# ViliamVadocz/takzero

Hardware: AMD Instinct MI355X
Metric: mcts_simulations_per_s (higher is better)
Workload: dtype f16

## Files before the change

takzero_amd/csrc/tz_capi.hip:

```cpp
#include <algorithm>
#include <array>
#include <cmath>
#include <cstdlib>
#include <cstring>
#include <vector>

#include "tz_math.h"
#include "tz_nn.h"

struct tz_search {
    SearchDev d;
    tz_net* net = nullptr;
    int device = 0;
    hipStream_t stream = nullptr;
    bool own_stream = false;
    float* noise_dev = nullptr;
    int noise_cap = 0;
    uint16_t* act_dev = nullptr;
    int32_t* i32_dev = nullptr;
    int8_t* i8_dev = nullptr;
    tz_root_info* info_dev = nullptr;
    void* child_dev = nullptr;
    size_t child_cap = 0;
    hipGraphExec_t graph[2] = {nullptr, nullptr};
// ... 106 lines not shown
            if (s->net) s->net->profile = v;
        }
    } restore{s, saved_net_profile};
    if (profile) {
        TZ_HIP(hipEventCreate(&e0));
        TZ_HIP(hipEventCreate(&e1));
        TZ_HIP(hipEventCreate(&e2));
        TZ_HIP(hipEventCreate(&e3));
        TZ_HIP(hipEventRecord(e0, s->stream));
    }
    if ((rc = tz_tree_descend(s->d, from_start, s->stream))) return rc;
    if ((rc = tz_tree_compact_leaves(s->d, s->stream))) return rc;
    if (profile) TZ_HIP(hipEventRecord(e1, s->stream));
    NetOut out{nullptr, 0, nullptr, nullptr};
    if (s->d.agent_kind == TZ_AGENT_NET) {
        if ((rc = tz_net_forward_device(s->net, s->d.leaf_env, s->d.nn_game, s->d.nn_count, 0, s->d.batch, s->stream, &out)))
            return rc;
    }
    if (profile) TZ_HIP(hipEventRecord(e2, s->stream));
    if ((rc = tz_tree_expand(s->d, out, s->stream))) return rc;
    if (profile) {
        TZ_HIP(hipEventRecord(e3, s->stream));
        s->tree_events.push_back({e0, e1});
        s->tree_events.push_back({e2, e3});
        s->steps++;
    }
    return TZ_OK;
}

int ensure_noise(tz_search* s, int amax) {
    if ((size_t)amax * s->d.batch <= (size_t)s->noise_cap) return TZ_OK;
// ... 742 lines not shown
```

takzero_amd/csrc/tz_engine.h:

```cpp
#pragma once
#include <hip/hip_runtime.h>
#include <stdint.h>

#include <string>
#include <vector>

#include "../../include/takzero_hip.h"

#define TZ_MAX_DEPTH 512

void tz_set_error(const std::string& msg);
int tz_fail(int code, const std::string& msg);
#define TZ_HIP(call)                                                                              \
    do {                                                                                          \
        hipError_t _e = (call);                                                                   \
        if (_e != hipSuccess)                                                                     \
            return tz_fail(TZ_EDEVICE, std::string(#call) + ": " + hipGetErrorString(_e));       \
    } while (0)

struct TreeArrays {
    uint8_t* eval_tag;
    uint32_t* eval_bits;
    uint32_t* visits;
    float* prob;
// ... 40 lines not shown
    float* prob;
    float* value;
    float* variance;
    uint8_t* bad;
    int32_t* count;
    int32_t* forwards;
    int32_t* offset;
    int32_t* index;
};

struct NetOut {
    const float* policy;
    int policy_stride;
    const float* value;
    const float* variance;
};

int tz_tree_descend(const SearchDev& s, bool from_start_nodes, hipStream_t st);
int tz_tree_compact_leaves(const SearchDev& s, hipStream_t st);
int tz_tree_expand(const SearchDev& s, const NetOut& out, hipStream_t st);
int tz_tree_apply_noise(const SearchDev& s, const float* noise_dev, int amax, float ratio, hipStream_t st);
int tz_tree_root_info(const SearchDev& s, tz_root_info* out_dev, hipStream_t st);
int tz_tree_root_children(const SearchDev& s, int amax, uint16_t* move_idx, uint32_t* visits, uint8_t* eval_tag,
                          uint32_t* eval_bits, float* logit, float* prob, float* std_dev, hipStream_t st);
int tz_tree_node(const SearchDev& s, int game, const uint16_t* path_dev, int len, uint32_t* out_words, int* status, int amax,
                 uint16_t* move_idx, uint32_t* visits, uint8_t* eval_tag, uint32_t* eval_bits, float* logit, float* prob, float* std_dev,
                 hipStream_t st);
int tz_tree_select_best(const SearchDev& s, uint16_t* out_dev, hipStream_t st);
int tz_tree_step(const SearchDev& s, const uint16_t* actions_dev, hipStream_t st);
int tz_tree_restart(const SearchDev& s, const int32_t* choice_dev, int8_t* terminal_dev, bool force_all,
                    bool with_opening_moves, hipStream_t st);
int tz_tree_reset_games(const SearchDev& s, const int32_t* idx_dev, int count, hipStream_t st);
// ... 8 lines not shown
```

takzero_amd/csrc/tz_nn.h:

```cpp
#pragma once
#include <string>
#include <vector>

#include "tz_engine.h"
#include "tz_ot.h"

struct ConvW {
    int taps = 0, cin = 0, cin_pad = 0, cout = 0, cout_pad = 0;
    uint16_t* w_mfma = nullptr;
    uint16_t* w_lo = nullptr;
    unsigned char* w8 = nullptr;
    float c8_scale = 0.0f;
    float* w_f32 = nullptr;
    float* bias = nullptr;
};

struct tz_net {
    int n = 0, nn = 0, arch = 0, device = 0, precision = 0, blocks = 0;
    int cin = 0, cin_pad = 0, pol_ch = 0, pol_stride = 0, ppt = 0;
    bool loaded = false, has_rnd = false, has_hash = false, has_ens = false;
    TensorStore store;
    uint64_t capture_gen = 0;
    ConvW conv_in, policy;
    std::vector<ConvW> res;
// ... 29 lines not shown
    void* dbg_buf = nullptr;
    int dbg_groups = 0;
    void* eval_host = nullptr;
    void* eval_dev = nullptr;
    size_t eval_bytes = 0;
    hipEvent_t ev0 = nullptr, ev1 = nullptr;
    std::vector<std::pair<hipEvent_t, hipEvent_t>> conv_events;
    bool profile = false;
    double conv_ms = 0.0;
    uint64_t conv_launches = 0;
};

int tz_net_ensure_batch(tz_net* net, int batch);
void tz_net_invalidate_captures(tz_net* net);
int tz_net_forward_device(tz_net* net, const tz_state* states_dev, const int32_t* game_index_dev,
                          const int32_t* count_dev, int count_host, int max_positions, hipStream_t st, NetOut* out);
int tz_nn_encode_planes(int n, int cin, const tz_state* states_dev, int count, float* planes_dev, hipStream_t st);
```

takzero_amd/csrc/tz_nn.hip:

```cpp
#include "tz_nn.h"
#include "tz_fp8.h"
#include "tz_fp6.h"
#include "tz_math.h"
#include <type_traits>
#include "tz_ot.h"

#include <algorithm>
#include <cmath>
#include <cstdio>
#include <cstdlib>
#include <cstring>
#include <atomic>
#include <map>
#include <memory>
#include <mutex>
#include <thread>

int tz_nn_launch_split(int sp, int n, const void* net_args, int max_positions, hipStream_t st);
int tz_nn_launch_c6(int n, const void* net_args, int max_positions, hipStream_t st);
size_t tz_nn_c6_seed_bytes(int n, int max_positions);

namespace {

typedef float f32x4 __attribute__((ext_vector_type(4)));
// ... 2353 lines not shown
    float ss = 0.f;
    for (int sq = 0; sq < NN; sq++) ss += part[sq];
#pragma unroll
    for (int k = 0; k < PER; k++) {
        const int i = l + k * 64;
        if (i < out_stride) out[(size_t)pos * out_stride + i] = (ET)(i < in_size ? x[k] / ss : 0.f);
    }
}

__global__ __launch_bounds__(64) void rnd_finish_kernel(const float* learn, const float* target, const float* ube,
                                                        const int32_t* count_dev, int count_host, int dim, int stride,
                                                        float rmin, float rmax, float* variance) {
    const int count = count_dev ? *count_dev : count_host;
    const int pos = blockIdx.x, l = threadIdx.x;
    if (pos >= count) return;
    float s = 0.f;
    for (int i = l; i < dim; i += 64) {
        const float d = learn[(size_t)pos * stride + i] - target[(size_t)pos * stride + i];
        s += d * d;
    }
    for (int d = 32; d >= 1; d >>= 1) s += __shfl_xor(s, d);
    if (l == 0) {
        float norm = (s - rmin) / (rmax - rmin);
        norm = fminf(fmaxf(norm, 0.f), 1.f) * 4.0f;
        variance[pos] = fminf(fmaxf(fmaxf(expf(ube[pos]), norm), 0.f), 4.f);
    }
}

__global__ void plain_variance_kernel(const float* ube, const float* local, const int32_t* count_dev, int count_host,
                                      float* variance) {
    const int count = count_dev ? *count_dev : count_host;
    const int pos = blockIdx.x * blockDim.x + threadIdx.x;
    if (pos >= count) return;
    const float loc = local ? local[pos] : 0.f;
    variance[pos] = fminf(fmaxf(fmaxf(expf(ube[pos]), loc), 0.f), 4.f);
}

__device__ __forceinline__ float ens_add(float x, float y) {
    _Pragma("clang fp contract(off)")
    return x + y;
}
// ... 685 lines not shown
    static bool attr_done[64] = {};
    int attr_dev = 0;
    TZ_HIP(hipGetDevice(&attr_dev));
    bool& attr_set = attr_done[attr_dev & 63];
    if (!attr_set) {
        TZ_HIP(hipFuncSetAttribute(reinterpret_cast<const void*>(kern), hipFuncAttributeMaxDynamicSharedMemorySize, (int)smem));
        attr_set = true;
    }
    dim3 grid((max_positions + P - 1) / P, n_blocks_y, a.groups > 1 ? a.groups : 1);
    hipLaunchKernelGGL(kern, grid, dim3(NW * 64), smem, st, a);
    hipError_t e = hipGetLastError();
    if (e != hipSuccess) return tz_fail(TZ_EDEVICE, std::string("conv launch: ") + hipGetErrorString(e));
    return TZ_OK;
}

int linear_grouped_bf16(int precision, const uint16_t* w, const float* bias, int groups, int cin_pad, int cout_pad, const void* in,
                        int in_stride, int in_z, void* out, int out_stride, int out_z, bool relu, bool out_f32,
                        const int32_t* count_dev, int count_host, int max_positions, hipStream_t st) {
    ConvArgs a;
    memset(&a, 0, sizeof a);
    a.in = in;
    a.count_dev = count_dev;
    a.count_host = count_host;
    a.w = w;
    a.bias = bias;
    a.out = out;
    a.cin_pad = cin_pad;
    a.kc_total = cin_pad / 32;
    a.ct_total = cout_pad / 16;
    a.out_stride = out_stride;
    a.cin_real = cin_pad;
    a.relu = relu;
    a.out_f32 = out_f32;
    a.in_stride = in_stride;
    a.groups = groups;
    a.in_z = in_z;
    a.w_z_frags = a.kc_total * a.ct_total;
    a.bias_z = cout_pad;
    a.out_z = out_z;
    if (max_positions <= 128) {
        if (prec_is_f16(precision)) return launch_conv<1, 32, 8, 2, 1, false, false, 0, 1, _Float16>(a, max_positions, cout_pad / 256, st);
        return launch_conv<1, 32, 8, 2, 1, false, false>(a, max_positions, cout_pad / 256, st);
    }
    if (prec_is_f16(precision)) return launch_conv<1, 128, 8, 2, 1, false, false, 0, 1, _Float16>(a, max_positions, cout_pad / 256, st);
    return launch_conv<1, 128, 8, 2, 1, false, false>(a, max_positions, cout_pad / 256, st);
}

template <int NB, typename ET>
int conv_board(const ConvArgs& a, int cout_pad, bool from_state, int max_positions, hipStream_t st) {
    constexpr int PA = ppt_for(NB), PB = ppt_small(NB);
    const bool wide = cout_pad % 256 == 0;
    const int by = wide ? cout_pad / 256 : cout_pad / 128;
    if (conv_cfg() == 0) {
        if (from_state) return launch_conv<NB, PA, 8, 2, 9, true, false, 0, 1, ET>(a, max_positions, by, st);
        if (wide) return launch_conv<NB, PA, 8, 2, 9, false, true, 0, 1, ET>(a, max_positions, by, st);
        return launch_conv<NB, PA, 8, 1, 9, false, true, 0, 1, ET>(a, max_positions, by, st);
    }
    if (from_state) return launch_conv<NB, PB, 4, 4, 9, true, false, 0, 1, ET>(a, max_positions, by, st);
// ... 429 lines not shown
        TZ_HIP(hipMalloc(&net->ens_act, rows * FILTERS * sizeof(float)));
        TZ_HIP(hipMalloc(&net->ens_values, (size_t)batch * ENS_HEADS * sizeof(float)));
    }
    if (net->has_rnd) {
        const size_t in_pad = (size_t)(net->cin * net->nn + 31) / 32 * 32;
        TZ_HIP(hipMalloc(&net->rnd_in, (size_t)batch * in_pad * esz));
        TZ_HIP(hipMalloc(&net->rnd_h1, (size_t)batch * 2048 * esz));
        TZ_HIP(hipMalloc(&net->rnd_h2, (size_t)batch * 2048 * esz));
        TZ_HIP(hipMalloc(&net->rnd_out, (size_t)2 * batch * 512 * sizeof(float)));
    }
    net->max_batch = batch;
    return TZ_OK;
}

int tz_net_forward_device(tz_net* net, const tz_state* states, const int32_t* gidx, const int32_t* count_dev,
                          int count_host, int max_positions, hipStream_t st, NetOut* out) {
    if (!net->loaded) return tz_fail(TZ_ESTATE, "network has no weights loaded");
    if (max_positions > net->max_batch) return tz_fail(TZ_EINVAL, "forward: batch exceeds the network's buffers");
    int rc;
    const bool bf = net->precision != TZ_PREC_F32;
    const int nn = net->nn;
    const bool need_planes = !bf;
    if (need_planes && (rc = encode(net, states, gidx, count_dev, count_host, max_positions, st))) return rc;
    void *x = net->act_a, *t = net->act_b, *y = net->act_c;
    const void* last = nullptr;
    const bool split = prec_is_split(net->precision);
    const int rnd_in_pad = (net->cin * nn + 31) / 32 * 32;
    const bool rnd_ahead = net->eval_split && net->has_rnd && bf && net->n == 5 && net->stream_rnd;
    auto rnd_mlp = [&](hipStream_t rs) -> int {
        const bool fused_wrote_it = net->blocks > 0 && net->tower_w && (net_fused_mode() == 2 || split) && net_fused_writes_rnd_input(net);
        switch (net->n) {
// ... 109 lines not shown
        last = fx;
    }
    if (net->has_ens) {
        if (!last) ensemble_heads_kernel<float><<<max_positions, 256, 0, st>>>(net->ens_act, net->ens_w, count_dev, count_host, net->ens_values, net->aux, net->ube, net->variance);
        else if (!bf) ensemble_heads_kernel<float><<<max_positions, 256, 0, st>>>((const float*)last, net->ens_w, count_dev, count_host, net->ens_values, net->aux, net->ube, net->variance);
        else if (prec_is_f16(net->precision))
            ensemble_heads_kernel<_Float16><<<max_positions, 256, 0, st>>>((const _Float16*)last, net->ens_w, count_dev, count_host, net->ens_values, net->aux, net->ube, net->variance);
        else ensemble_heads_kernel<__bf16><<<max_positions, 256, 0, st>>>((const __bf16*)last, net->ens_w, count_dev, count_host, net->ens_values, net->aux, net->ube, net->variance);
    } else if (net->has_rnd) {
        const int in_size = net->cin * nn, in_pad = (in_size + 31) / 32 * 32;
        float* outs[2] = {net->rnd_out, net->rnd_out + (size_t)net->max_batch * 512};
        if (bf) {
            if (!rnd_ahead && (rc = rnd_mlp(st))) return rc;
            if (rnd_ahead) TZ_HIP(hipStreamWaitEvent(st, net->ev_rnd, 0));
            float* o = net->rnd_out;
            rnd_finish_kernel<<<max_positions, 64, 0, st>>>(o, o + 512, net->ube, count_dev, count_host, 512, 1024, net->rnd_min,
                                                            net->rnd_max, net->variance);
        } else {
            rnd_prep_kernel<float><<<max_positions, 64, 0, st>>>(net->planes, count_dev, count_host, in_size, in_pad, (float*)net->rnd_in);
            for (int a = 0; a < 2; a++) {
                if ((rc = conv_f32(net, net->rnd[a][0], (float*)net->rnd_in, in_pad, count_dev, count_host, max_positions, nullptr,
                                   (float*)net->rnd_h1, 1024, true, false, st)))
                    return rc;
                if ((rc = conv_f32(net, net->rnd[a][1], (float*)net->rnd_h1, 1024, count_dev, count_host, max_positions, nullptr,
                                   (float*)net->rnd_h2, 1024, true, false, st)))
                    return rc;
                if ((rc = conv_f32(net, net->rnd[a][2], (float*)net->rnd_h2, 1024, count_dev, count_host, max_positions, nullptr,
                                   outs[a], 512, false, false, st)))
                    return rc;
            }
        }
        if (!bf)
            rnd_finish_kernel<<<max_positions, 64, 0, st>>>(outs[0], outs[1], net->ube, count_dev, count_host, 512, 512, net->rnd_min,
                                                            net->rnd_max, net->variance);
    } else if (net->has_hash) {
        if ((rc = launch_hash_state(net, states, gidx, count_dev, count_host, max_positions, nullptr, st))) return rc;
        plain_variance_kernel<<<(max_positions + 255) / 256, 256, 0, st>>>(net->ube, net->aux, count_dev, count_host, net->variance);
    } else {
        plain_variance_kernel<<<(max_positions + 255) / 256, 256, 0, st>>>(net->ube, nullptr, count_dev, count_host, net->variance);
    }
    hipError_t e = hipGetLastError();
    if (e != hipSuccess) return tz_fail(TZ_EDEVICE, std::string("forward launch: ") + hipGetErrorString(e));
    out->policy = net->policy_out;
    out->policy_stride = net->pol_stride;
    out->value = net->value;
    out->variance = net->variance;
    return TZ_OK;
}

extern "C" {

int tz_device_count(void) {
    int n = 0;
    if (hipGetDeviceCount(&n) != hipSuccess) return 0;
    return n;
}

int tz_net_create(int board_n, int arch, int device_id, int precision, int blocks, tz_net** out) {
    if (!out) return tz_fail(TZ_EINVAL, "tz_net_create: null out");
    int n = board_n;
    if (arch == TZ_ARCH_NET5) n = 5;
// ... 942 lines not shown
```

takzero_amd/csrc/tz_tree.hip:

```cpp
#include "tz_engine.h"
#include "tz_math.h"
#include "tz_tak_dev.h"

using namespace tzd;

namespace {

struct Ev {
    uint32_t tag, bits;
};
__device__ __forceinline__ Ev ev_value(float v) { return Ev{TZ_EVAL_VALUE, tz_float_to_bits(v)}; }
__device__ __forceinline__ bool ev_known(Ev e) { return e.tag != TZ_EVAL_VALUE; }
__device__ __forceinline__ Ev ev_negate(Ev e) {
    switch (e.tag) {
        case TZ_EVAL_VALUE: return ev_value(-tz_bits_to_float(e.bits));
        case TZ_EVAL_WIN: return Ev{TZ_EVAL_LOSS, e.bits + 1};
        case TZ_EVAL_DRAW: return Ev{TZ_EVAL_DRAW, e.bits + 1};
        default: return Ev{TZ_EVAL_WIN, e.bits + 1};
    }
}
__device__ __forceinline__ float ev_to_f32(Ev e) {
    const float base = tz_powif(TZ_DISCOUNT, e.tag == TZ_EVAL_VALUE ? 0 : (int)e.bits);
    const float x = e.tag == TZ_EVAL_VALUE ? tz_bits_to_float(e.bits)
                    : e.tag == TZ_EVAL_WIN ? 1.0f
// ... 70 lines not shown
#pragma unroll
    for (int d = 32; d >= 1; d >>= 1) {
        Ev o{(uint32_t)__shfl_xor((int)best.tag, d), (uint32_t)__shfl_xor((int)best.bits, d)};
        const int oi = __shfl_xor(best_i, d);
        if (oi != 0x7fffffff) {
            const int c = best_i == 0x7fffffff ? -1 : ev_cmp(o, best);
            if (c < 0 || (c == 0 && oi < best_i)) {
                best = o;
                best_i = oi;
            }
        }
    }
    min_out = best;
}

__device__ void backup(const SearchDev& s, size_t base, const uint32_t* tnode, const uint32_t* tvis, int leaf_level,
                       Ev child_eval, float child_var, Ev stored) {
    for (int lvl = leaf_level - 1; lvl >= 0; lvl--) {
        const uint32_t node = tnode[lvl], below = tnode[lvl + 1];
        Ev ev{s.t.eval_tag[base + node], s.t.eval_bits[base + node]};
        float sd = s.t.std_dev[base + node];
        const uint32_t c0 = s.t.child0[base + node];
        const int nc = s.t.nchild[base + node];
        Ev mn;
        bool all_known;
        children_min_allknown(s, base, c0, nc, below, stored, mn, all_known);
        if (child_eval.tag == TZ_EVAL_LOSS || all_known) {
            ev = ev_negate(mn);
            sd = 0.0f;
        }
        Ev up;
        float up_var;
        if (ev_known(ev)) {
            up = ev;
            up_var = sd * sd;
        } else {
            const float negated = ev_to_notnan(ev_negate(child_eval));
            const float n = (float)tvis[lvl];
// ... 9 lines not shown
            s.t.eval_bits[base + node] = ev.bits;
            s.t.std_dev[base + node] = sd;
        }
        stored = ev;
        child_eval = up;
        child_var = up_var;
    }
}

template <int N, int RULE>
struct SelectRow {
    static constexpr int LEN = RULE == TZ_SELECT_IMPROVED ? (N <= 5 ? TZ_MAX_ACTIONS : TZ_MAX_ACTIONS_6) : 0;
};

template <int N, int RULE>
__device__ __forceinline__ int forward_walk(const SearchDev& s, size_t base, tz_state& env, uint32_t* tnode, uint32_t* tvis,
                                            uint32_t node, float beta, int& depth, Ev& known, float* prow) {
    const int l = lane_id();
    for (;;) {
        const uint32_t vis = s.t.visits[base + node] + 1;
        if (l == 0) {
            s.t.visits[base + node] = vis;
            tnode[depth] = node;
            tvis[depth] = vis;
        }
        depth++;
        const Ev ev{s.t.eval_tag[base + node], s.t.eval_bits[base + node]};
        const int nc = s.t.nchild[base + node];
        if (ev_known(ev) && ev.bits == 0) {
            known = ev;
            return 0;
        }
// ... 118 lines not shown
            if (oi >= 0 && (best_i < 0 || os > best_score || (os == best_score && oi > best_i))) {
                best_score = os;
                best_i = oi;
            }
        }
        if (best_i < 0) {
            if (l == 0) atomicMax(s.error_flag, 4);
            return 2;
        }
        node = c0 + (uint32_t)best_i;
        apply_move<N>(&env, s.t.action[base + node]);
        __syncthreads();
    }
}

template <int N, int RULE>
__global__ __launch_bounds__(64) void descend_kernel(SearchDev s, int from_start) {
    constexpr int NN = N * N;
    const int g = blockIdx.x, l = lane_id();
    __shared__ tz_state env;
    __shared__ uint32_t tnode[TZ_MAX_DEPTH];
    __shared__ uint32_t tvis[TZ_MAX_DEPTH];
    __shared__ uint8_t reach[NN * 4];
    float* prow = nullptr;
    if constexpr (RULE == TZ_SELECT_IMPROVED) {
        __shared__ float row[SelectRow<N, RULE>::LEN];
        prow = row;
    }
    load_state(&env, &s.env[g]);
    const size_t base = slab_base(s, s.bank[g], g);
    uint32_t node = 0;
    float beta = s.betas[g];
    if (from_start) {
        node = (uint32_t)s.start_node[g];
        beta = 0.0f;
    }
    __syncthreads();
    if (from_start && node != 0) {
        apply_move<N>(&env, s.t.action[base + node]);
        __syncthreads();
    }
    int depth = 0;
    Ev known{0, 0};
    const int kind = forward_walk<N, RULE>(s, base, env, tnode, tvis, node, beta, depth, known, prow);
    __syncthreads();
    if (kind == 0) {
        backup(s, base, tnode, tvis, depth - 1, known, 0.0f, known);
        if (l == 0) {
            s.leaf_kind[g] = 0;
            s.traj_len[g] = 0;
        }
        return;
    }
    if (kind == 2) {
        if (l == 0) {
            s.leaf_kind[g] = 0;
            s.traj_len[g] = 0;
        }
        return;
    }
    uint16_t* acts = s.leaf_act + (size_t)g * s.max_actions;
    const int nact = gen_moves<N>(&env, reach, acts, s.max_actions);
// ... 25 lines not shown
        __syncthreads();
        int off = carry;
        for (int i = 0; i < w; i++) off += wsum[i];
        if (f) s.nn_game[off + incl - 1] = g;
        __syncthreads();
        if (tid == 1023) carry = off + incl;
        __syncthreads();
    }
    if (tid == 0) {
        *s.nn_count = carry;
        s.counters[0] += (unsigned long long)s.batch;
        s.counters[1] += (unsigned long long)carry;
    }
}

template <int N>
__global__ __launch_bounds__(64) void expand_kernel(SearchDev s, NetOut out) {
    constexpr int NN = N * N;
    const int slot = blockIdx.x, l = lane_id();
    if (slot >= *s.nn_count) return;
    const int g = s.nn_game[slot];
    extern __shared__ __attribute__((aligned(16))) unsigned char smem[];
    uint32_t* tnode = reinterpret_cast<uint32_t*>(smem);
    uint32_t* tvis = tnode + TZ_MAX_DEPTH;
    float* lg = reinterpret_cast<float*>(tvis + TZ_MAX_DEPTH);
    float* ex = lg + s.max_actions;
    const size_t base = slab_base(s, s.bank[g], g);
    const int len = (int)s.traj_len[g];
    for (int i = l; i < len; i += 64) {
        const uint32_t nd = s.traj[(size_t)g * TZ_MAX_DEPTH + i];
        tnode[i] = nd;
        tvis[i] = s.t.visits[base + nd];
    }
    const int nact = s.leaf_nact[g];
    const uint16_t* acts = s.leaf_act + (size_t)g * s.max_actions;
    float value = 0.0f, variance = 0.0f;
    if (s.agent_kind == TZ_AGENT_NET) {
        value = out.value[slot];
        variance = out.variance[slot];
    } else if (s.agent_kind == TZ_AGENT_SIMPLE) {
        __shared__ tz_state le;
        load_state(&le, &s.leaf_env[g]);
        __syncthreads();
        const int fd = flat_diff<N>(&le) - s.half_komi / 2;
        value = (float)fd / (float)NN;
        if (le.to_move == 1) value = -value;
    }
    bool nan = false;
    float mx = -3.4028235e38f;
    for (int i = l; i < nact; i += 64) {
        const int a = acts[i];
        float x;
        if (s.agent_kind == TZ_AGENT_NET) {
            x = out.policy[((size_t)slot * NN + (a % NN)) * out.policy_stride + a / NN];
// ... 45 lines not shown
        s.t.nchild[ci] = 0;
        s.t.action[ci] = acts[i];
    }
    if (l == 0) {
        s.t.eval_bits[base + leaf] = tz_float_to_bits(mean);
        s.t.std_dev[base + leaf] = sd;
        if (full) {
            atomicAdd(&s.counters[2], 1ull);
        } else {
            s.alloc[g] = c0 + (uint32_t)nact;
            s.t.child0[base + leaf] = c0;
            s.t.nchild[base + leaf] = (uint16_t)nact;
        }
    }
    __syncthreads();
    backup(s, base, tnode, tvis, len - 1, ev_value(value * TZ_DISCOUNT), variance * TZ_DISCOUNT * TZ_DISCOUNT, ev_value(mean));
}

template <int N, int RULE>
__global__ __launch_bounds__(64) void descend_batch_kernel(SearchDev s, LeafBatchDev b) {
    constexpr int NN = N * N;
    const int g = blockIdx.x, l = lane_id();
    __shared__ tz_state root_env;
    __shared__ tz_state env;
    __shared__ uint32_t tnode[TZ_MAX_DEPTH];
    __shared__ uint32_t tvis[TZ_MAX_DEPTH];
    __shared__ uint8_t reach[NN * 4];
    float* prow = nullptr;
    if constexpr (RULE == TZ_SELECT_IMPROVED) {
        __shared__ float row[SelectRow<N, RULE>::LEN];
        prow = row;
    }
    load_state(&root_env, &s.env[g]);
    const size_t base = slab_base(s, s.bank[g], g);
    const float beta = s.betas[g];
    int collected = 0, forwards = 0;
    __syncthreads();
    for (int f = 0; f < 4 * b.leaves && collected < b.leaves; f++) {
        load_state(&env, &root_env);
        __syncthreads();
        int depth = 0;
        Ev known{0, 0};
        const int kind = forward_walk<N, RULE>(s, base, env, tnode, tvis, 0, beta, depth, known, prow);
        __syncthreads();
        forwards++;
        if (kind == 2) break;
        if (kind == 0) {
            backup(s, base, tnode, tvis, depth - 1, known, 0.0f, known);
        } else {
            const size_t slot = (size_t)g * b.leaves + collected;
            uint16_t* acts = b.act + slot * s.max_actions;
            const int nact = gen_moves<N>(&env, reach, acts, s.max_actions);
            if (nact > s.max_actions && l == 0) atomicMax(s.error_flag, 3);
            {
                const uint32_t* a = reinterpret_cast<const uint32_t*>(&env);
                uint32_t* d = reinterpret_cast<uint32_t*>(&b.env[slot]);
                for (int i = l; i < (int)(sizeof(tz_state) / 4); i += 64) d[i] = a[i];
            }
            for (int i = l; i < depth; i += 64) b.traj[slot * TZ_MAX_DEPTH + i] = tnode[i];
            if (l == 0) {
                b.nact[slot] = (uint16_t)(nact > s.max_actions ? s.max_actions : nact);
                b.traj_len[slot] = (uint32_t)depth;
            }
// ... 104 lines not shown
    float sum = 0.0f;
    for (int i = 0; i < nact; i++) sum = sum + ex[i];
    float* lo = b.logit + (size_t)slot * s.max_actions;
    float* po = b.prob + (size_t)slot * s.max_actions;
    for (int i = l; i < nact; i += 64) {
        lo[i] = lg[i];
        po[i] = ex[i] / sum;
    }
    if (l == 0) {
        b.value[slot] = value;
        b.variance[slot] = variance;
        b.bad[slot] = 0;
    }
}

__global__ __launch_bounds__(64) void expand_batch_kernel(SearchDev s, LeafBatchDev b) {
    const int g = blockIdx.x, l = lane_id();
    __shared__ uint32_t tnode[TZ_MAX_DEPTH];
    __shared__ uint32_t tvis[TZ_MAX_DEPTH];
    const size_t base = slab_base(s, s.bank[g], g);
    const int count = b.count[g];
    for (int j = 0; j < count; j++) {
        const size_t slot = (size_t)g * b.leaves + j;
        if (b.bad[slot]) return;
        const int len = (int)b.traj_len[slot];
        for (int i = l; i < len; i += 64) {
            const uint32_t nd = b.traj[slot * TZ_MAX_DEPTH + i];
            tnode[i] = nd;
            tvis[i] = s.t.visits[base + nd];
        }
// ... 31 lines not shown
                s.t.action[ci] = acts[i];
            }
        }
        if (l == 0) {
            s.t.eval_bits[base + leaf] = tz_float_to_bits(mean);
            s.t.std_dev[base + leaf] = sd;
            if (full) {
                atomicAdd(&s.counters[2], 1ull);
            } else if (!again) {
                s.alloc[g] = c0 + (uint32_t)nact;
                s.t.child0[base + leaf] = c0;
                s.t.nchild[base + leaf] = (uint16_t)nact;
            }
        }
        __syncthreads();
        backup(s, base, tnode, tvis, len - 1, ev_value(value * TZ_DISCOUNT), variance * TZ_DISCOUNT * TZ_DISCOUNT, ev_value(mean));
        __threadfence_block();
        __syncthreads();
    }
}

__global__ __launch_bounds__(64) void noise_kernel(SearchDev s, const float* noise, int amax, float ratio) {
    const int g = blockIdx.x, l = lane_id();
    const size_t base = slab_base(s, s.bank[g], g);
    const int nc = s.t.nchild[base];
    const bool known = s.t.eval_tag[base] != TZ_EVAL_VALUE;
    if (nc == 0 && !known) {
        if (l == 0) atomicMax(s.error_flag, 6);
        return;
    }
    const uint32_t c0 = s.t.child0[base];
// ... 436 lines not shown
    if (!a || !b || !out || n <= 0) return tz_fail(TZ_EINVAL, "tz_device_math: bad argument");
    float *da = nullptr, *db = nullptr, *dout = nullptr;
    TZ_HIP(hipMalloc(&da, n * 4));
    TZ_HIP(hipMalloc(&db, n * 4));
    TZ_HIP(hipMalloc(&dout, n * 4));
    TZ_HIP(hipMemcpy(da, a, n * 4, hipMemcpyHostToDevice));
    TZ_HIP(hipMemcpy(db, b, n * 4, hipMemcpyHostToDevice));
    device_math_kernel<<<(n + 255) / 256, 256>>>(op, da, db, dout, n);
    TZ_HIP(hipMemcpy(out, dout, n * 4, hipMemcpyDeviceToHost));
    (void)hipFree(da);
    (void)hipFree(db);
    (void)hipFree(dout);
    return TZ_OK;
}

int tz_tree_descend(const SearchDev& s, bool from_start_nodes, hipStream_t st) {
    TZ_DISPATCH_N(s.n, TZ_DISPATCH_RULE(s.select_rule, (descend_kernel<NB, RB><<<s.batch, 64, 0, st>>>(s, from_start_nodes ? 1 : 0))));
    TZ_LAUNCH_CHECK();
    return TZ_OK;
}
int tz_tree_compact_leaves(const SearchDev& s, hipStream_t st) {
    compact_kernel<<<1, 1024, 0, st>>>(s);
    TZ_LAUNCH_CHECK();
    return TZ_OK;
}
int tz_tree_expand(const SearchDev& s, const NetOut& out, hipStream_t st) {
    const size_t smem = 2 * TZ_MAX_DEPTH * sizeof(uint32_t) + 2 * (size_t)s.max_actions * sizeof(float);
    TZ_DISPATCH_N(s.n, (expand_kernel<NB><<<s.batch, 64, smem, st>>>(s, out)));
    TZ_LAUNCH_CHECK();
    return TZ_OK;
}
int tz_tree_apply_noise(const SearchDev& s, const float* noise_dev, int amax, float ratio, hipStream_t st) {
    noise_kernel<<<s.batch, 64, 0, st>>>(s, noise_dev, amax, ratio);
    TZ_LAUNCH_CHECK();
    return TZ_OK;
}
int tz_tree_root_info(const SearchDev& s, tz_root_info* out_dev, hipStream_t st) {
    TZ_DISPATCH_N(s.n, (root_info_kernel<NB><<<s.batch, 64, 0, st>>>(s, out_dev)));
    TZ_LAUNCH_CHECK();
    return TZ_OK;
}
int tz_tree_root_children(const SearchDev& s, int amax, uint16_t* move_idx, uint32_t* visits, uint8_t* eval_tag,
                          uint32_t* eval_bits, float* logit, float* prob, float* std_dev, hipStream_t st) {
// ... 40 lines not shown
    set_start_kernel<<<(s.batch + 255) / 256, 256, 0, st>>>(s, child_index_dev);
    TZ_LAUNCH_CHECK();
    return TZ_OK;
}
int tz_tree_gumbel_root_fixup(const SearchDev& s, hipStream_t st) {
    gumbel_fixup_kernel<<<s.batch, 64, 0, st>>>(s);
    TZ_LAUNCH_CHECK();
    return TZ_OK;
}
int tz_tree_principal_variation(const SearchDev& s, int game, uint16_t* moves_dev, int cap, int* len_dev, hipStream_t st) {
    principal_variation_kernel<<<1, 64, 0, st>>>(s, game, moves_dev, cap, len_dev);
    TZ_LAUNCH_CHECK();
    return TZ_OK;
}
int tz_tree_descend_batch(const SearchDev& s, const LeafBatchDev& b, hipStream_t st) {
    TZ_DISPATCH_N(s.n, TZ_DISPATCH_RULE(s.select_rule, (descend_batch_kernel<NB, RB><<<s.batch, 64, 0, st>>>(s, b))));
    TZ_LAUNCH_CHECK();
    return TZ_OK;
}
int tz_tree_compact_batch(const SearchDev& s, const LeafBatchDev& b, hipStream_t st) {
    compact_batch_kernel<<<1, 1024, 0, st>>>(s, b);
    TZ_LAUNCH_CHECK();
    return TZ_OK;
}
int tz_tree_expand_batch(const SearchDev& s, const LeafBatchDev& b, const NetOut& out, hipStream_t st) {
    const size_t smem = 2 * (size_t)s.max_actions * sizeof(float);
    TZ_DISPATCH_N(s.n, (leaf_policy_kernel<NB><<<s.batch * b.leaves, 64, smem, st>>>(s, b, out)));
    TZ_LAUNCH_CHECK();
    expand_batch_kernel<<<s.batch, 64, 0, st>>>(s, b);
    TZ_LAUNCH_CHECK();
    return TZ_OK;
}
```

Measured before the change: 1.436 million.

## Restructure tree descent, backup prefetch, fuse RND variance into expand, smaller conv tiles

The tree walk now carries each chosen child's header through the wavefront shuffle reduction and loads two children per lane per iteration, so it no longer re-reads the selected node from global memory. Backup preloads ancestor node fields in parallel across lanes and then broadcasts them with shuffles instead of reading them serially. The RND variance finish kernel is folded into the expand kernel, which saves one launch per step. Grouped linear layers use 64-row tiles when the workgroup count fits within the CU count. The old path stays available behind the TZ_TREE_V1 environment variable, at the cost of duplicated kernel instantiations and more code complexity.

```diff
diff --git a/takzero_amd/csrc/tz_capi.hip b/takzero_amd/csrc/tz_capi.hip
--- a/takzero_amd/csrc/tz_capi.hip
+++ b/takzero_amd/csrc/tz_capi.hip
@@ -144,7 +144,8 @@
     if (profile) TZ_HIP(hipEventRecord(e1, s->stream));
     NetOut out{nullptr, 0, nullptr, nullptr};
     if (s->d.agent_kind == TZ_AGENT_NET) {
-        if ((rc = tz_net_forward_device(s->net, s->d.leaf_env, s->d.nn_game, s->d.nn_count, 0, s->d.batch, s->stream, &out)))
+        if ((rc = tz_net_forward_device(s->net, s->d.leaf_env, s->d.nn_game, s->d.nn_count, 0, s->d.batch, s->stream, &out,
+                                        s->net->has_rnd && !tz_tree_v1())))
             return rc;
     }
     if (profile) TZ_HIP(hipEventRecord(e2, s->stream));
diff --git a/takzero_amd/csrc/tz_engine.h b/takzero_amd/csrc/tz_engine.h
--- a/takzero_amd/csrc/tz_engine.h
+++ b/takzero_amd/csrc/tz_engine.h
@@ -78,8 +78,31 @@
     int policy_stride;
     const float* value;
     const float* variance;
+    const float* rnd_learn = nullptr;
+    const float* rnd_target = nullptr;
+    const float* rnd_ube = nullptr;
+    float* variance_out = nullptr;
+    int rnd_stride = 0, rnd_dim = 0;
+    float rnd_min = 0.0f, rnd_max = 0.0f;
 };
 
+#ifdef __HIPCC__
+__device__ __forceinline__ float tz_rnd_variance(const float* learn, const float* target, float ube, int dim, float rmin, float rmax) {
+#pragma clang fp contract(fast)
+    const int l = threadIdx.x & 63;
+    float s = 0.f;
+    for (int i = l; i < dim; i += 64) {
+        const float d = learn[i] - target[i];
+        s += d * d;
+    }
+    for (int d = 32; d >= 1; d >>= 1) s += __shfl_xor(s, d);
+    float norm = (s - rmin) / (rmax - rmin);
+    norm = fminf(fmaxf(norm, 0.f), 1.f) * 4.0f;
+    return fminf(fmaxf(fmaxf(expf(ube), norm), 0.f), 4.f);
+}
+#endif
+
+bool tz_tree_v1();
 int tz_tree_descend(const SearchDev& s, bool from_start_nodes, hipStream_t st);
 int tz_tree_compact_leaves(const SearchDev& s, hipStream_t st);
 int tz_tree_expand(const SearchDev& s, const NetOut& out, hipStream_t st);
diff --git a/takzero_amd/csrc/tz_nn.h b/takzero_amd/csrc/tz_nn.h
--- a/takzero_amd/csrc/tz_nn.h
+++ b/takzero_amd/csrc/tz_nn.h
@@ -67,5 +67,6 @@
 int tz_net_ensure_batch(tz_net* net, int batch);
 void tz_net_invalidate_captures(tz_net* net);
 int tz_net_forward_device(tz_net* net, const tz_state* states_dev, const int32_t* game_index_dev,
-                          const int32_t* count_dev, int count_host, int max_positions, hipStream_t st, NetOut* out);
+                          const int32_t* count_dev, int count_host, int max_positions, hipStream_t st, NetOut* out,
+                          bool finish_rnd_later = false);
 int tz_nn_encode_planes(int n, int cin, const tz_state* states_dev, int count, float* planes_dev, hipStream_t st);
diff --git a/takzero_amd/csrc/tz_nn.hip b/takzero_amd/csrc/tz_nn.hip
--- a/takzero_amd/csrc/tz_nn.hip
+++ b/takzero_amd/csrc/tz_nn.hip
@@ -2391,17 +2391,8 @@
     const int count = count_dev ? *count_dev : count_host;
     const int pos = blockIdx.x, l = threadIdx.x;
     if (pos >= count) return;
-    float s = 0.f;
-    for (int i = l; i < dim; i += 64) {
-        const float d = learn[(size_t)pos * stride + i] - target[(size_t)pos * stride + i];
-        s += d * d;
-    }
-    for (int d = 32; d >= 1; d >>= 1) s += __shfl_xor(s, d);
-    if (l == 0) {
-        float norm = (s - rmin) / (rmax - rmin);
-        norm = fminf(fmaxf(norm, 0.f), 1.f) * 4.0f;
-        variance[pos] = fminf(fmaxf(fmaxf(expf(ube[pos]), norm), 0.f), 4.f);
-    }
+    const float v = tz_rnd_variance(learn + (size_t)pos * stride, target + (size_t)pos * stride, ube[pos], dim, rmin, rmax);
+    if (l == 0) variance[pos] = v;
 }
 
 __global__ void plain_variance_kernel(const float* ube, const float* local, const int32_t* count_dev, int count_host,
@@ -3117,6 +3108,15 @@
     return TZ_OK;
 }
 
+int device_cu_count() {
+    static int cus[64] = {};
+    int dev = 0;
+    if (hipGetDevice(&dev) != hipSuccess) return 0;
+    int& n = cus[dev & 63];
+    if (n == 0 && (hipDeviceGetAttribute(&n, hipDeviceAttributeMultiprocessorCount, dev) != hipSuccess || n <= 0)) n = -1;
+    return n > 0 ? n : 0;
+}
+
 int linear_grouped_bf16(int precision, const uint16_t* w, const float* bias, int groups, int cin_pad, int cout_pad, const void* in,
                         int in_stride, int in_z, void* out, int out_stride, int out_z, bool relu, bool out_f32,
                         const int32_t* count_dev, int count_host, int max_positions, hipStream_t st) {
@@ -3145,6 +3145,11 @@
         if (prec_is_f16(precision)) return launch_conv<1, 32, 8, 2, 1, false, false, 0, 1, _Float16>(a, max_positions, cout_pad / 256, st);
         return launch_conv<1, 32, 8, 2, 1, false, false>(a, max_positions, cout_pad / 256, st);
     }
+    const int wgs128 = (max_positions + 127) / 128 * (cout_pad / 256) * (groups > 1 ? groups : 1);
+    if (!tz_tree_v1() && wgs128 <= device_cu_count()) {
+        if (prec_is_f16(precision)) return launch_conv<1, 64, 8, 2, 1, false, false, 0, 1, _Float16>(a, max_positions, cout_pad / 256, st);
+        return launch_conv<1, 64, 8, 2, 1, false, false>(a, max_positions, cout_pad / 256, st);
+    }
     if (prec_is_f16(precision)) return launch_conv<1, 128, 8, 2, 1, false, false, 0, 1, _Float16>(a, max_positions, cout_pad / 256, st);
     return launch_conv<1, 128, 8, 2, 1, false, false>(a, max_positions, cout_pad / 256, st);
 }
@@ -3604,7 +3609,7 @@
 }
 
 int tz_net_forward_device(tz_net* net, const tz_state* states, const int32_t* gidx, const int32_t* count_dev,
-                          int count_host, int max_positions, hipStream_t st, NetOut* out) {
+                          int count_host, int max_positions, hipStream_t st, NetOut* out, bool finish_rnd_later) {
     if (!net->loaded) return tz_fail(TZ_ESTATE, "network has no weights loaded");
     if (max_positions > net->max_batch) return tz_fail(TZ_EINVAL, "forward: batch exceeds the network's buffers");
     int rc;
@@ -3744,8 +3749,9 @@
             if (!rnd_ahead && (rc = rnd_mlp(st))) return rc;
             if (rnd_ahead) TZ_HIP(hipStreamWaitEvent(st, net->ev_rnd, 0));
             float* o = net->rnd_out;
-            rnd_finish_kernel<<<max_positions, 64, 0, st>>>(o, o + 512, net->ube, count_dev, count_host, 512, 1024, net->rnd_min,
-                                                            net->rnd_max, net->variance);
+            if (!finish_rnd_later)
+                rnd_finish_kernel<<<max_positions, 64, 0, st>>>(o, o + 512, net->ube, count_dev, count_host, 512, 1024, net->rnd_min,
+                                                                net->rnd_max, net->variance);
         } else {
             rnd_prep_kernel<float><<<max_positions, 64, 0, st>>>(net->planes, count_dev, count_host, in_size, in_pad, (float*)net->rnd_in);
             for (int a = 0; a < 2; a++) {
@@ -3775,6 +3781,15 @@
     out->policy_stride = net->pol_stride;
     out->value = net->value;
     out->variance = net->variance;
+    const bool later = finish_rnd_later && net->has_rnd && bf;
+    out->rnd_learn = later ? net->rnd_out : nullptr;
+    out->rnd_target = later ? net->rnd_out + 512 : nullptr;
+    out->rnd_ube = later ? net->ube : nullptr;
+    out->variance_out = later ? net->variance : nullptr;
+    out->rnd_stride = later ? 1024 : 0;
+    out->rnd_dim = later ? 512 : 0;
+    out->rnd_min = net->rnd_min;
+    out->rnd_max = net->rnd_max;
     return TZ_OK;
 }
 
diff --git a/takzero_amd/csrc/tz_tree.hip b/takzero_amd/csrc/tz_tree.hip
--- a/takzero_amd/csrc/tz_tree.hip
+++ b/takzero_amd/csrc/tz_tree.hip
@@ -108,14 +108,36 @@
     min_out = best;
 }
 
+template <bool V1>
 __device__ void backup(const SearchDev& s, size_t base, const uint32_t* tnode, const uint32_t* tvis, int leaf_level,
                        Ev child_eval, float child_var, Ev stored) {
+    uint32_t p_tag = 0, p_bits = 0, p_c0 = 0, p_nc = 0;
+    float p_sd = 0.0f;
+    if (!V1 && lane_id() < leaf_level) {
+        const size_t pi = base + tnode[lane_id()];
+        p_tag = s.t.eval_tag[pi];
+        p_bits = s.t.eval_bits[pi];
+        p_sd = s.t.std_dev[pi];
+        p_c0 = s.t.child0[pi];
+        p_nc = s.t.nchild[pi];
+    }
     for (int lvl = leaf_level - 1; lvl >= 0; lvl--) {
         const uint32_t node = tnode[lvl], below = tnode[lvl + 1];
-        Ev ev{s.t.eval_tag[base + node], s.t.eval_bits[base + node]};
-        float sd = s.t.std_dev[base + node];
-        const uint32_t c0 = s.t.child0[base + node];
-        const int nc = s.t.nchild[base + node];
+        Ev ev;
+        float sd;
+        uint32_t c0;
+        int nc;
+        if (!V1 && lvl < 64) {
+            ev = Ev{(uint32_t)__shfl((int)p_tag, lvl), (uint32_t)__shfl((int)p_bits, lvl)};
+            sd = __shfl(p_sd, lvl);
+            c0 = (uint32_t)__shfl((int)p_c0, lvl);
+            nc = __shfl((int)p_nc, lvl);
+        } else {
+            ev = Ev{s.t.eval_tag[base + node], s.t.eval_bits[base + node]};
+            sd = s.t.std_dev[base + node];
+            c0 = s.t.child0[base + node];
+            nc = s.t.nchild[base + node];
+        }
         Ev mn;
         bool all_known;
         children_min_allknown(s, base, c0, nc, below, stored, mn, all_known);
@@ -155,8 +177,8 @@
 };
 
 template <int N, int RULE>
-__device__ __forceinline__ int forward_walk(const SearchDev& s, size_t base, tz_state& env, uint32_t* tnode, uint32_t* tvis,
-                                            uint32_t node, float beta, int& depth, Ev& known, float* prow) {
+__device__ __forceinline__ int forward_walk_v1(const SearchDev& s, size_t base, tz_state& env, uint32_t* tnode, uint32_t* tvis,
+                                               uint32_t node, float beta, int& depth, Ev& known, float* prow) {
     const int l = lane_id();
     for (;;) {
         const uint32_t vis = s.t.visits[base + node] + 1;
@@ -305,7 +327,224 @@
     }
 }
 
+struct Hdr {
+    uint32_t visits, tag, bits, nchild, child0, action;
+};
+struct Child {
+    Hdr h;
+    float prob, sd;
+};
+__device__ __forceinline__ Child load_child(const SearchDev& s, size_t ci) {
+    Child c;
+    c.h.tag = s.t.eval_tag[ci];
+    c.h.bits = s.t.eval_bits[ci];
+    c.h.visits = s.t.visits[ci];
+    c.prob = s.t.prob[ci];
+    c.sd = s.t.std_dev[ci];
+    c.h.nchild = s.t.nchild[ci];
+    c.h.child0 = s.t.child0[ci];
+    c.h.action = s.t.action[ci];
+    return c;
+}
+
 template <int N, int RULE>
+__device__ __forceinline__ int forward_walk(const SearchDev& s, size_t base, tz_state& env, uint32_t* tnode, uint32_t* tvis,
+                                            uint32_t node, float beta, int& depth, Ev& known, float* prow) {
+    const int l = lane_id();
+    Hdr h;
+    h.visits = s.t.visits[base + node];
+    h.tag = s.t.eval_tag[base + node];
+    h.bits = s.t.eval_bits[base + node];
+    h.nchild = s.t.nchild[base + node];
+    h.child0 = s.t.child0[base + node];
+    h.action = 0;
+    for (;;) {
+        const uint32_t vis = h.visits + 1;
+        if (l == 0) {
+            s.t.visits[base + node] = vis;
+            tnode[depth] = node;
+            tvis[depth] = vis;
+        }
+        depth++;
+        const Ev ev{h.tag, h.bits};
+        const int nc = (int)h.nchild;
+        if (ev_known(ev) && ev.bits == 0) {
+            known = ev;
+            return 0;
+        }
+        if (nc == 0 && !ev_known(ev)) {
+            const int t = terminal<N>(&env);
+            if (t != TZ_TERMINAL_NONE) {
+                known = Ev{(uint32_t)(t == TZ_TERMINAL_WIN ? TZ_EVAL_WIN : t == TZ_TERMINAL_LOSS ? TZ_EVAL_LOSS : TZ_EVAL_DRAW), 0};
+                if (l == 0) {
+                    s.t.eval_tag[base + node] = (uint8_t)known.tag;
+                    s.t.eval_bits[base + node] = 0;
+                    s.t.std_dev[base + node] = 0.0f;
+                }
+                return 0;
+            }
+            return 1;
+        }
+        if (depth >= TZ_MAX_DEPTH) {
+            if (l == 0) atomicMax(s.error_flag, 2);
+            return 2;
+        }
+        const uint32_t c0 = h.child0;
+        const float parent = (float)vis;
+        const bool parent_loss = ev.tag == TZ_EVAL_LOSS;
+        float best_score = 0.0f;
+        int best_i = -1;
+        Hdr best_h{0, 0, 0, 0, 0, 0};
+        if constexpr (RULE == TZ_SELECT_PUCT) {
+            const float er = tz_logf(((1.0f + parent) + 500.0f) / 500.0f) + 4.0f;
+            const float sq = sqrtf(parent);
+            auto consider = [&](int i, const Child& c) {
+                const Ev ce{c.h.tag, c.h.bits};
+                if (!(parent_loss || ce.tag != TZ_EVAL_WIN)) return;
+                const float q = ev_to_notnan(ev_negate(ce));
+                const float puct = ((er * c.prob) * sq) / (1.0f + (float)c.h.visits);
+                const float score = (q + puct) + c.sd * beta;
+                if (best_i < 0 || !(score < best_score)) {
+                    best_score = score;
+                    best_i = i;
+                    best_h = c.h;
+                }
+            };
+            for (int i = l; i < nc; i += 128) {
+                const bool two = i + 64 < nc;
+                const Child a = load_child(s, base + c0 + i);
+                const Child b = load_child(s, base + c0 + (two ? i + 64 : i));
+                consider(i, a);
+                if (two) consider(i + 64, b);
+            }
+        } else if constexpr (RULE == TZ_SELECT_UCT) {
+            const float lnp = tz_logf(parent);
+            bool nan = false;
+            auto consider = [&](int i, const Child& c) {
+                const Ev ce{c.h.tag, c.h.bits};
+                if (!(parent_loss || ce.tag != TZ_EVAL_WIN)) return;
+                const float q = ev_to_notnan(ev_negate(ce));
+                const float uct = 1.0f * sqrtf(lnp / (float)c.h.visits);
+                const float score = (q + uct) + c.sd * beta;
+                nan = nan || !(score == score);
+                if (best_i < 0 || !(score < best_score)) {
+                    best_score = score;
+                    best_i = i;
+                    best_h = c.h;
+                }
+            };
+            for (int i = l; i < nc; i += 128) {
+                const bool two = i + 64 < nc;
+                const Child a = load_child(s, base + c0 + i);
+                const Child b = load_child(s, base + c0 + (two ? i + 64 : i));
+                consider(i, a);
+                if (two) consider(i + 64, b);
+            }
+            if (__any(nan)) {
+                if (l == 0) atomicMax(s.error_flag, 8);
+                return 2;
+            }
+        } else {
+            if (nc > SelectRow<N, RULE>::LEN) {
+                if (l == 0) atomicMax(s.error_flag, 3);
+                return 2;
+            }
+            uint32_t vm = 0;
+            for (int i = l; i < nc; i += 64) {
+                const uint32_t v = s.t.visits[base + c0 + i];
+                vm = v > vm ? v : vm;
+            }
+#pragma unroll
+            for (int d = 32; d >= 1; d >>= 1) {
+                const uint32_t o = (uint32_t)__shfl_xor((int)vm, d);
+                vm = o > vm ? o : vm;
+            }
+            const float sqv = sqrtf((float)vm);
+            bool nan = false;
+            float mx = -3.4028235e38f;
+            for (int i = l; i < nc; i += 64) {
+                const size_t ci = base + c0 + i;
+                const Ev ce{s.t.eval_tag[ci], s.t.eval_bits[ci]};
+                const bool needs_init = s.t.nchild[ci] == 0 && !ev_known(ce);
+                const float completed = ev_to_f32(needs_init ? ev : ev_negate(ce));
+                const float p = ((completed + s.t.std_dev[ci] * 0.0f) * sqv) + s.t.logit[ci];
+                nan = nan || !(p == p);
+                prow[i] = p;
+                mx = p > mx ? p : mx;
+            }
+#pragma unroll
+            for (int d = 32; d >= 1; d >>= 1) {
+                const float o = __shfl_xor(mx, d);
+                mx = o > mx ? o : mx;
+            }
+            if (__any(nan)) {
+                if (l == 0) atomicMax(s.error_flag, 8);
+                return 2;
+            }
+            for (int i = l; i < nc; i += 64) prow[i] = tz_expf(prow[i] - mx);
+            __syncthreads();
+            float sum = 0.0f;
+            for (int i = 0; i < nc; i++) sum = sum + prow[i];
+            const float denom = (float)(vis + 1u);
+            for (int i = l; i < nc; i += 64) {
+                const size_t ci = base + c0 + i;
+                Hdr ch;
+                ch.tag = s.t.eval_tag[ci];
+                ch.bits = s.t.eval_bits[ci];
+                ch.visits = s.t.visits[ci];
+                ch.nchild = s.t.nchild[ci];
+                ch.child0 = s.t.child0[ci];
+                ch.action = s.t.action[ci];
+                if (!(parent_loss || ch.tag != TZ_EVAL_WIN)) continue;
+                const float score = prow[i] / sum - (float)ch.visits / denom;
+                nan = nan || !(score == score);
+                if (best_i < 0 || !(score < best_score)) {
+                    best_score = score;
+                    best_i = i;
+                    best_h = ch;
+                }
+            }
+            if (__any(nan)) {
+                if (l == 0) atomicMax(s.error_flag, 8);
+                return 2;
+            }
+        }
+#pragma unroll
+        for (int d = 32; d >= 1; d >>= 1) {
+            const float os = __shfl_xor(best_score, d);
+            const int oi = __shfl_xor(best_i, d);
+            Hdr oh;
+            oh.visits = (uint32_t)__shfl_xor((int)best_h.visits, d);
+            oh.tag = (uint32_t)__shfl_xor((int)best_h.tag, d);
+            oh.bits = (uint32_t)__shfl_xor((int)best_h.bits, d);
+            oh.nchild = (uint32_t)__shfl_xor((int)best_h.nchild, d);
+            oh.child0 = (uint32_t)__shfl_xor((int)best_h.child0, d);
+            oh.action = (uint32_t)__shfl_xor((int)best_h.action, d);
+            if (oi >= 0 && (best_i < 0 || os > best_score || (os == best_score && oi > best_i))) {
+                best_score = os;
+                best_i = oi;
+                best_h = oh;
+            }
+        }
+        if (best_i < 0) {
+            if (l == 0) atomicMax(s.error_flag, 4);
+            return 2;
+        }
+        node = c0 + (uint32_t)best_i;
+        h = best_h;
+        apply_move<N>(&env, (int)h.action);
+        __syncthreads();
+    }
+}
+
+template <int N, int RULE, bool V1>
+__device__ __forceinline__ int forward_walk_ab(const SearchDev& s, size_t base, tz_state& env, uint32_t* tnode, uint32_t* tvis,
+                                               uint32_t node, float beta, int& depth, Ev& known, float* prow) {
+    if constexpr (V1) return forward_walk_v1<N, RULE>(s, base, env, tnode, tvis, node, beta, depth, known, prow);
+    else return forward_walk<N, RULE>(s, base, env, tnode, tvis, node, beta, depth, known, prow);
+}
+
+template <int N, int RULE, bool V1>
 __global__ __launch_bounds__(64) void descend_kernel(SearchDev s, int from_start) {
     constexpr int NN = N * N;
     const int g = blockIdx.x, l = lane_id();
@@ -333,10 +572,10 @@
     }
     int depth = 0;
     Ev known{0, 0};
-    const int kind = forward_walk<N, RULE>(s, base, env, tnode, tvis, node, beta, depth, known, prow);
+    const int kind = forward_walk_ab<N, RULE, V1>(s, base, env, tnode, tvis, node, beta, depth, known, prow);
     __syncthreads();
     if (kind == 0) {
-        backup(s, base, tnode, tvis, depth - 1, known, 0.0f, known);
+        backup<V1>(s, base, tnode, tvis, depth - 1, known, 0.0f, known);
         if (l == 0) {
             s.leaf_kind[g] = 0;
             s.traj_len[g] = 0;
@@ -392,7 +631,7 @@
     }
 }
 
-template <int N>
+template <int N, bool V1>
 __global__ __launch_bounds__(64) void expand_kernel(SearchDev s, NetOut out) {
     constexpr int NN = N * N;
     const int slot = blockIdx.x, l = lane_id();
@@ -415,7 +654,13 @@
     float value = 0.0f, variance = 0.0f;
     if (s.agent_kind == TZ_AGENT_NET) {
         value = out.value[slot];
-        variance = out.variance[slot];
+        if (out.rnd_learn) {
+            variance = tz_rnd_variance(out.rnd_learn + (size_t)slot * out.rnd_stride, out.rnd_target + (size_t)slot * out.rnd_stride,
+                                       out.rnd_ube[slot], out.rnd_dim, out.rnd_min, out.rnd_max);
+            if (l == 0) out.variance_out[slot] = variance;
+        } else {
+            variance = out.variance[slot];
+        }
     } else if (s.agent_kind == TZ_AGENT_SIMPLE) {
         __shared__ tz_state le;
         load_state(&le, &s.leaf_env[g]);
@@ -491,10 +736,10 @@
         }
     }
     __syncthreads();
-    backup(s, base, tnode, tvis, len - 1, ev_value(value * TZ_DISCOUNT), variance * TZ_DISCOUNT * TZ_DISCOUNT, ev_value(mean));
-}
-
-template <int N, int RULE>
+    backup<V1>(s, base, tnode, tvis, len - 1, ev_value(value * TZ_DISCOUNT), variance * TZ_DISCOUNT * TZ_DISCOUNT, ev_value(mean));
+}
+
+template <int N, int RULE, bool V1>
 __global__ __launch_bounds__(64) void descend_batch_kernel(SearchDev s, LeafBatchDev b) {
     constexpr int NN = N * N;
     const int g = blockIdx.x, l = lane_id();
@@ -518,12 +763,12 @@
         __syncthreads();
         int depth = 0;
         Ev known{0, 0};
-        const int kind = forward_walk<N, RULE>(s, base, env, tnode, tvis, 0, beta, depth, known, prow);
+        const int kind = forward_walk_ab<N, RULE, V1>(s, base, env, tnode, tvis, 0, beta, depth, known, prow);
         __syncthreads();
         forwards++;
         if (kind == 2) break;
         if (kind == 0) {
-            backup(s, base, tnode, tvis, depth - 1, known, 0.0f, known);
+            backup<V1>(s, base, tnode, tvis, depth - 1, known, 0.0f, known);
         } else {
             const size_t slot = (size_t)g * b.leaves + collected;
             uint16_t* acts = b.act + slot * s.max_actions;
@@ -658,6 +903,7 @@
     }
 }
 
+template <bool V1>
 __global__ __launch_bounds__(64) void expand_batch_kernel(SearchDev s, LeafBatchDev b) {
     const int g = blockIdx.x, l = lane_id();
     __shared__ uint32_t tnode[TZ_MAX_DEPTH];
@@ -719,7 +965,7 @@
             }
         }
         __syncthreads();
-        backup(s, base, tnode, tvis, len - 1, ev_value(value * TZ_DISCOUNT), variance * TZ_DISCOUNT * TZ_DISCOUNT, ev_value(mean));
+        backup<V1>(s, base, tnode, tvis, len - 1, ev_value(value * TZ_DISCOUNT), variance * TZ_DISCOUNT * TZ_DISCOUNT, ev_value(mean));
         __threadfence_block();
         __syncthreads();
     }
@@ -1186,8 +1432,17 @@
     return TZ_OK;
 }
 
+bool tz_tree_v1() {
+    static const bool v1 = [] {
+        const char* e = getenv("TZ_TREE_V1");
+        return e && *e && *e != '0';
+    }();
+    return v1;
+}
+
 int tz_tree_descend(const SearchDev& s, bool from_start_nodes, hipStream_t st) {
-    TZ_DISPATCH_N(s.n, TZ_DISPATCH_RULE(s.select_rule, (descend_kernel<NB, RB><<<s.batch, 64, 0, st>>>(s, from_start_nodes ? 1 : 0))));
+    TZ_DISPATCH_N(s.n, TZ_DISPATCH_RULE(s.select_rule, (tz_tree_v1() ? descend_kernel<NB, RB, true><<<s.batch, 64, 0, st>>>(s, from_start_nodes ? 1 : 0)
+                                                                     : descend_kernel<NB, RB, false><<<s.batch, 64, 0, st>>>(s, from_start_nodes ? 1 : 0))));
     TZ_LAUNCH_CHECK();
     return TZ_OK;
 }
@@ -1198,7 +1453,7 @@
 }
 int tz_tree_expand(const SearchDev& s, const NetOut& out, hipStream_t st) {
     const size_t smem = 2 * TZ_MAX_DEPTH * sizeof(uint32_t) + 2 * (size_t)s.max_actions * sizeof(float);
-    TZ_DISPATCH_N(s.n, (expand_kernel<NB><<<s.batch, 64, smem, st>>>(s, out)));
+    TZ_DISPATCH_N(s.n, (tz_tree_v1() ? expand_kernel<NB, true><<<s.batch, 64, smem, st>>>(s, out) : expand_kernel<NB, false><<<s.batch, 64, smem, st>>>(s, out)));
     TZ_LAUNCH_CHECK();
     return TZ_OK;
 }
@@ -1269,7 +1524,8 @@
     return TZ_OK;
 }
 int tz_tree_descend_batch(const SearchDev& s, const LeafBatchDev& b, hipStream_t st) {
-    TZ_DISPATCH_N(s.n, TZ_DISPATCH_RULE(s.select_rule, (descend_batch_kernel<NB, RB><<<s.batch, 64, 0, st>>>(s, b))));
+    TZ_DISPATCH_N(s.n, TZ_DISPATCH_RULE(s.select_rule, (tz_tree_v1() ? descend_batch_kernel<NB, RB, true><<<s.batch, 64, 0, st>>>(s, b)
+                                                                     : descend_batch_kernel<NB, RB, false><<<s.batch, 64, 0, st>>>(s, b))));
     TZ_LAUNCH_CHECK();
     return TZ_OK;
 }
@@ -1282,7 +1538,8 @@
     const size_t smem = 2 * (size_t)s.max_actions * sizeof(float);
     TZ_DISPATCH_N(s.n, (leaf_policy_kernel<NB><<<s.batch * b.leaves, 64, smem, st>>>(s, b, out)));
     TZ_LAUNCH_CHECK();
-    expand_batch_kernel<<<s.batch, 64, 0, st>>>(s, b);
-    TZ_LAUNCH_CHECK();
-    return TZ_OK;
-}
+    if (tz_tree_v1()) expand_batch_kernel<true><<<s.batch, 64, 0, st>>>(s, b);
+    else expand_batch_kernel<false><<<s.batch, 64, 0, st>>>(s, b);
+    TZ_LAUNCH_CHECK();
+    return TZ_OK;
+}
```

New measurement: 1.425 million. About the same (-0.7%).
